# freemvmt/two-towers-overlords

Hardware: NVIDIA B200
Metric: train_triplets_per_sec (higher is better)
Workload: dtype f32 (bf16x3 tensor-core projection)

## Files before the change

### two-towers-overlords_b200/csrc/tt_chain_sm100.cu

```cuda
#include <stdlib.h>

#include "tt_ptx.cuh"
#include "tt_step_ws.cuh"
#include "tt_tma.cuh"

namespace tt {

namespace {

using namespace ptx;

constexpr int BM = 128, BN = 128, BK = 64;
constexpr int kMaxStages = 6;
constexpr int kAcc = 4;
constexpr int kEpiThreads = 256;
constexpr int kThreads = 64 + kEpiThreads;
constexpr uint32_t kABytes = BM * BK * 2, kBBytes = BN * BK * 2, kStageBytes = kABytes + kBBytes;
constexpr int kSplitPad = 66;
constexpr int kRowStage = 3072;
constexpr int kTermPitch = 48;
constexpr int kTermBlock = 32 * kTermPitch;
constexpr int kF32Pitch = 80;
constexpr int kCsBytes = 2 * 8 * 64 * 4;
constexpr int kStagingBytes = kCsBytes  + 8 * kRowStage  + 64;
static_assert(2 * 64 * kSplitPad * 2 <= 8 * kRowStage, "split tiles overlay the row staging");
constexpr size_t chain_smem(int stages) { return (size_t)stages * kStageBytes + 1024 + 256 + kStagingBytes; }
constexpr float kCosEps = 1e-8f;
constexpr long long kSpinLimit = 4000000000ll;

enum { T_S = 0, T_T, T_F1, T_F2L, T_DZ, T_DX, T_DW2, T_DW1, T_G, T_COUNT };

struct TowerMaps {
  CUtensorMap x[3], w1[3];
  CUtensorMap h[2], w2[2];
  CUtensorMap dy[2];
  CUtensorMap dz[2], w1k[2];
  CUtensorMap dyk[2], hk[2];
  CUtensorMap dzk[2], xk[2];
};

struct SplitJobC {
  const float* X;
  bf16 *hi, *lo, *lo2;
  int R, C;
  int f4_0;
};

struct alignas(64) ChainParams {
  TowerMaps tm[2];
  int B, H, P, RTB, NC, NCH, NCF, ldt, dcol;
  int pairs, terms, pairs1, terms1;
  int kcb, nch[2], kbt[2];
  int off[T_COUNT + 1];
  int stages, n_sj, n_split_f4, n_split_f4_w1;
  int nS;
  int krot;
  int use_pdl;
  SplitJobC sj[6];
  float margin, inv_batch, grad_scale;
  const float *b1[2], *b2[2];
  float *h, *y, *dy, *dz1, *dxhat, *stats, *loss;
  bf16 *h_hi, *h_lo, *dy_hi, *dy_lo, *dz_hi, *dz_lo;
  float *part2, *part1;
  float *dW1[2], *db1[2], *dW2[2], *db2[2];
  float *stat_part, *cs1, *cs2, *hinge_part, *ybuf;
  unsigned* ctr;
  int n_counters;
  double* adam_state;
  float *adam_p, *adam_g, *adam_m, *adam_v;
  float lr, beta1, beta2, eps;
  unsigned total_signals, dw2_signals;
  unsigned long long* trace;
};

__device__ __forceinline__ unsigned ld_acquire(const unsigned* p) {
  unsigned v;
  asm volatile("ld.acquire.gpu.global.u32 %0, [%1];" : "=r"(v) : "l"(p) : "memory");
  return v;
}
__device__ __forceinline__ void signal(unsigned* p) {
  asm volatile("red.release.gpu.global.add.u32 [%0], 1;" ::"l"(p) : "memory");
}
__device__ __forceinline__ void fence_proxy_async() { asm volatile("fence.proxy.async;" ::: "memory"); }
__device__ __forceinline__ unsigned ld_relaxed(const unsigned* p) {
  unsigned v;
  asm volatile("ld.relaxed.gpu.global.u32 %0, [%1];" : "=r"(v) : "l"(p) : "memory");
  return v;
}
__device__ __forceinline__ void wait_counter(const unsigned* p, unsigned target) {
  if (ld_relaxed(p) < target) {
    const long long t0 = clock64();
    while (ld_relaxed(p) < target) {
      __nanosleep(32);
      if (clock64() - t0 > kSpinLimit) __trap();
    }
  }
  asm volatile("fence.acq_rel.gpu;" ::: "memory");
}
__device__ __forceinline__ void epi_bar() { asm volatile("bar.sync 1, 256;" ::: "memory"); }

struct Task {
  int type, i;
};
__device__ __forceinline__ Task decode(const ChainParams& p, int idx) {
  int t = 0;
#pragma unroll
  for (int k = 1; k < T_COUNT; ++k)
    if (idx >= p.off[k]) t = k;
  return Task{t, idx - p.off[t]};
}

struct RowTile {
  int r, seg, t, trow, grow, valid;
};
__device__ __forceinline__ RowTile row_tile(const ChainParams& p, int u) {
  RowTile rt;
  rt.r = u / 3;
  rt.seg = u - 3 * rt.r;
  rt.t = rt.seg != 0;
  rt.trow = (rt.seg == 2 ? p.B : 0) + rt.r * BM;
  rt.grow = rt.seg * p.B + rt.r * BM;
  rt.valid = min(BM, p.B - rt.r * BM);
  return rt;
}

struct Sub {
  const CUtensorMap *a, *b;
  int terms, pairs, m0, n0, kb0, nkb;
  int bn;
  int amn, bmn;
};
__device__ __forceinline__ int n_subs(int type) {
  return (type == T_S || type == T_T || type == T_G) ? 0 : 1;
}

__device__ __forceinline__ void dw_chunk(const ChainParams& p, int ci, int& t, int& j) {
  t = ci >= p.nch[0];
  j = ci - (t ? p.nch[0] : 0);
}

__device__ __forceinline__ Sub get_sub(const ChainParams& p, Task tk, int k) {
  Sub s;
  s.terms = p.terms;
  s.pairs = p.pairs;
  s.kb0 = 0;
  s.bn = BN;
  s.amn = s.bmn = 0;
  switch (tk.type) {
    case T_F1: {
      const RowTile rt = row_tile(p, tk.i / p.NC);
      s.a = p.tm[rt.t].x; s.b = p.tm[rt.t].w1;
      s.terms = p.terms1; s.pairs = p.pairs1;
// ... 99 lines not shown
  for (int j = 0; j < 2; ++j) {
    const float keep = h4 ? b[2 + j] : b[j], send = h4 ? b[j] : b[2 + j];
    c[j] = keep + __shfl_xor_sync(0xffffffffu, send, 4);
  }
  const float keep = h2 ? c[1] : c[0], send = h2 ? c[0] : c[1];
  float d = keep + __shfl_xor_sync(0xffffffffu, send, 2);
  d += __shfl_xor_sync(0xffffffffu, d, 1);
  return d;
}

__device__ __forceinline__ void store16(float* dst, const float (&v)[16]) {
  float4* d = reinterpret_cast<float4*>(dst);
#pragma unroll
  for (int j = 0; j < 4; ++j) d[j] = make_float4(v[4 * j], v[4 * j + 1], v[4 * j + 2], v[4 * j + 3]);
}

__device__ __forceinline__ void split16(const float (&v)[16], bf16 (&hi)[16], bf16 (&lo)[16]) {
#pragma unroll
  for (int j = 0; j < 16; ++j) split_bf16(v[j], hi[j], lo[j]);
}
__device__ __forceinline__ void stage16(uint8_t* blk, int lane, const bf16 (&x)[16]) {
  uint4* d = reinterpret_cast<uint4*>(blk + lane * kTermPitch);
  d[0] = reinterpret_cast<const uint4*>(x)[0];
  d[1] = reinterpret_cast<const uint4*>(x)[1];
}
__device__ __forceinline__ void flush16(const uint8_t* blk, int lane, bf16* g, size_t row0, int n, int ld, int vr) {
#pragma unroll
  for (int it = 0; it < 2; ++it) {
    const int r = it * 16 + (lane >> 1), sg = lane & 1;
    if (r < vr)
      *reinterpret_cast<uint4*>(g + (row0 + r) * ld + n + sg * 8) =
          *reinterpret_cast<const uint4*>(blk + r * kTermPitch + sg * 16);
  }
}
__device__ __forceinline__ void stage_f32(uint8_t* blk, int lane, const float (&v)[16]) {
  float4* d = reinterpret_cast<float4*>(blk + lane * kF32Pitch);
#pragma unroll
  for (int j = 0; j < 4; ++j) d[j] = make_float4(v[4 * j], v[4 * j + 1], v[4 * j + 2], v[4 * j + 3]);
}
__device__ __forceinline__ void flush_f32(const uint8_t* blk, int lane, float* g, size_t row0, int n, size_t ld, int vr) {
#pragma unroll
  for (int it = 0; it < 4; ++it) {
    const int r = it * 8 + (lane >> 2), sg = lane & 3;
    if (r < vr)
      *reinterpret_cast<float4*>(g + (row0 + r) * ld + n + sg * 4) =
          *reinterpret_cast<const float4*>(blk + r * kF32Pitch + sg * 16);
  }
}

struct EpiCtx {
  uint32_t tmem_base;
  uint64_t *acc_full, *acc_empty;
  float* cs_s;
  bf16* sp_s;
  float* hs_s;
  uint8_t* rs;
  int we, q, hf, lane, tid;
  int ab;
  uint32_t aph;
  unsigned long long* trace;
  int tslot, tidx;
};

__device__ __forceinline__ void trace_ev(EpiCtx& e, int kind) {
  if (e.trace && e.tid == 0 && e.tslot < kTraceSlots) {
    unsigned long long t;
    asm volatile("mov.u64 %0, %globaltimer;" : "=l"(t));
    e.trace[e.tslot * 2] = ((unsigned long long)e.tidx << 2) | (unsigned long long)kind;
    e.trace[e.tslot * 2 + 1] = t;
    ++e.tslot;
  }
}

__device__ __forceinline__ uint32_t acc_addr(const EpiCtx& e, int buf, int chunk) {
  return e.tmem_base + ((uint32_t)(e.q * 32) << 16) + (uint32_t)(buf * BN + e.hf * 64 + chunk * 16);
}
__device__ __forceinline__ void acc_advance(EpiCtx& e, int n) {
  e.ab += n;
  if (e.ab >= kAcc) {
    e.ab -= kAcc;
    e.aph ^= 1u;
  }
}
__device__ __forceinline__ void publish(const EpiCtx& e) {
  fence_proxy_async();
  __threadfence();
  epi_bar();
}

__device__ __forceinline__ void stage_cs(const EpiCtx& e, int slot, int chunk, float d) {
  if ((e.lane & 1) == 0) e.cs_s[(slot * 8 + e.we) * 64 + chunk * 16 + (e.lane >> 1)] = d;
}
__device__ __forceinline__ float reduce_cs(const EpiCtx& e, int slot, int col, int cw = 64) {
  const int hf = col / cw, cc = col - hf * cw;
  float s = 0.f;
#pragma unroll
  for (int quarter = 0; quarter < 4; ++quarter) s += e.cs_s[(slot * 8 + hf * 4 + ((quarter - 2) & 3)) * 64 + cc];
  return s;
}

__device__ __forceinline__ uint32_t pack_bf16(bf16 a, bf16 b) {
  return (uint32_t)__bfloat16_as_ushort(a) | ((uint32_t)__bfloat16_as_ushort(b) << 16);
}

__device__ void epi_split(const ChainParams& p, EpiCtx& e, int task_i) {
  const int nS = p.nS;
  if (task_i == 0 && e.tid == 0 && p.adam_state) {
    const double t = p.adam_state[0];
    p.adam_state[0] = t + 1.0;
    p.adam_state[1] = (t == 0.0 ? 1.0 : p.adam_state[1]) * (double)p.beta1;
    p.adam_state[2] = (t == 0.0 ? 1.0 : p.adam_state[2]) * (double)p.beta2;
  }
  constexpr int U = 4;
  const int gstride = nS * kEpiThreads;
  for (int part = 0; part < 2; ++part) {
    const int lo_i = part ? p.n_split_f4_w1 : 0, hi_i = part ? p.n_split_f4 : p.n_split_f4_w1;
    for (int base = lo_i + task_i * kEpiThreads + e.tid; base < hi_i; base += U * gstride) {
      float4 v[U];
      int ji[U], li[U];
#pragma unroll
      for (int u = 0; u < U; ++u) {
        const int i = base + u * gstride;
        ji[u] = -1;
        if (i < hi_i) {
          int j = 0;
          for (int k = 1; k < p.n_sj; ++k)
            if (i >= p.sj[k].f4_0) j = k;
          ji[u] = j;
          li[u] = i - p.sj[j].f4_0;
          v[u] = __ldg(reinterpret_cast<const float4*>(p.sj[j].X) + li[u]);
        }
      }
#pragma unroll
      for (int u = 0; u < U; ++u) {
        if (ji[u] < 0) continue;
        const SplitJobC& J = p.sj[ji[u]];
        const float x[4] = {v[u].x, v[u].y, v[u].z, v[u].w};
        bf16 h[4], l[4];
#pragma unroll
        for (int k = 0; k < 4; ++k) split_bf16(x[k], h[k], l[k]);
        reinterpret_cast<uint2*>(J.hi)[li[u]] = make_uint2(pack_bf16(h[0], h[1]), pack_bf16(h[2], h[3]));
        reinterpret_cast<uint2*>(J.lo)[li[u]] = make_uint2(pack_bf16(l[0], l[1]), pack_bf16(l[2], l[3]));
        if (J.lo2) {
          bf16 m[4];
#pragma unroll
          for (int k = 0; k < 4; ++k)
            m[k] = __float2bfloat16_rn((x[k] - __bfloat162float(h[k])) - __bfloat162float(l[k]));
          reinterpret_cast<uint2*>(J.lo2)[li[u]] = make_uint2(pack_bf16(m[0], m[1]), pack_bf16(m[2], m[3]));
        }
      }
    }
    if (part == 0) {
      publish(e);
      if (e.tid == 0) signal(p.ctr + 0);
    }
  }
  publish(e);
  if (e.tid == 0) signal(p.ctr + 2);
}

__device__ __forceinline__ int warp_valid_rows(const EpiCtx& e, int valid) { return max(0, min(32, valid - e.q * 32)); }

__device__ void epi_f1(const ChainParams& p, EpiCtx& e, int task_i) {
  const RowTile rt = row_tile(p, task_i / p.NC);
  const int n0 = (task_i % p.NC) * BN;
  mbar_wait(&e.acc_full[e.ab], e.aph);
  tc_fence_after();
  trace_ev(e, 2);
  const int row = e.q * 32 + e.lane;
  const bool ok = row < rt.valid;
  const int vr = warp_valid_rows(e, rt.valid);
  const size_t wrow0 = (size_t)rt.grow + e.q * 32;
  const float* bias = p.b1[rt.t];
  for (int ch = 0; ch < 4; ++ch) {
    const int n = n0 + e.hf * 64 + ch * 16;
    if (n >= p.P) break;
    float v[16];
    tmem_ld16(acc_addr(e, e.ab, ch), v);
#pragma unroll
    for (int j = 0; j < 16; ++j) v[j] = fmaxf(v[j] + __ldg(bias + n + j), 0.f);
    alignas(16) bf16 hi[16], lo[16];
    split16(v, hi, lo);
    stage16(e.rs, e.lane, hi);
    stage16(e.rs + kTermBlock, e.lane, lo);
    if (ok && p.h) store16(p.h + (wrow0 + e.lane) * p.P + n, v);
    __syncwarp();
    flush16(e.rs, e.lane, p.h_hi, wrow0, n, p.P, vr);
    flush16(e.rs + kTermBlock, e.lane, p.h_lo, wrow0, n, p.P, vr);
    __syncwarp();
  }
  tc_fence_before();
  mbar_arrive(&e.acc_empty[e.ab]);
  acc_advance(e, 1);
  publish(e);
  if (e.tid == 0) signal(h_ready(p) + rt.seg * p.RTB + rt.r);
}

__device__ void epi_f2l(const ChainParams& p, EpiCtx& e, int task_i) {
  const int seg = task_i % 3, rc = task_i / 3, r = rc / p.NCF, c = rc % p.NCF, n0 = c * 64;
  const int valid = min(BM, p.B - r * BM);
  const int row = e.q * 32 + e.lane;
  const bool ok = row < valid;
  const int vr = warp_valid_rows(e, valid);
  const int trip = r * BM + row;
  const size_t wrow0 = (size_t)seg * p.B + (size_t)r * BM + e.q * 32;
  mbar_wait(&e.acc_full[e.ab], e.aph);
  tc_fence_after();
  trace_ev(e, 2);
  const uint32_t accb = e.tmem_base + ((uint32_t)(e.q * 32) << 16) + (uint32_t)(e.ab * BN + e.hf * 32);
  const float* bias = p.b2[seg != 0];
  float* X = p.ybuf + (size_t)rc * 3 * 64 * 128;
  float own[32];
#pragma unroll
  for (int ch = 0; ch < 2; ++ch) {
    const int col = e.hf * 32 + ch * 16;
    float v[16];
    tmem_ld16(accb + ch * 16, v);
#pragma unroll
    for (int j = 0; j < 16; ++j) {
      v[j] += __ldg(bias + n0 + col + j);
      own[ch * 16 + j] = v[j];
      X[((size_t)(seg * 64 + col + j)) * 128 + row] = v[j];
    }
    if (p.y && ok) store16(p.y + ((size_t)seg * p.B + trip) * p.P + n0 + col, v);
  }
  tc_fence_before();
  mbar_arrive(&e.acc_empty[e.ab]);
  acc_advance(e, 1);
  __threadfence();
  epi_bar();
  if (e.tid == 0) {
    signal(y_ready(p) + rc);
    wait_counter(y_ready(p) + rc, 3u);
  }
  epi_bar();
  const int s1 = seg == 0 ? 1 : 0, s2 = seg == 2 ? 1 : 2;
  float f1[32], f2[32];
  {
    const float* x1 = X + (size_t)(s1 * 64 + e.hf * 32) * 128 + row;
    const float* x2 = X + (size_t)(s2 * 64 + e.hf * 32) * 128 + row;
#pragma unroll
    for (int j = 0; j < 32; ++j) {
      f1[j] = __ldcg(x1 + (size_t)j * 128);
      f2[j] = __ldcg(x2 + (size_t)j * 128);
    }
  }
  float qq = 0.f, pp = 0.f, nn = 0.f, qp = 0.f, qn = 0.f;
#pragma unroll
  for (int j = 0; j < 32; ++j) {
    const float a = seg == 0 ? own[j] : f1[j];
    const float b = seg == 0 ? f1[j] : (seg == 1 ? own[j] : f2[j]);
    const float d = seg == 2 ? own[j] : f2[j];
    qq = fmaf(a, a, qq);
    pp = fmaf(b, b, pp);
    nn = fmaf(d, d, nn);
    qp = fmaf(a, b, qp);
    qn = fmaf(a, d, qn);
  }
  const int nslots = p.NCF;
  float* xs = e.cs_s;
  if (seg == 0 && e.hf == 1) {
    xs[row] = qq; xs[128 + row] = pp; xs[256 + row] = nn; xs[384 + row] = qp; xs[512 + row] = qn;
  }
  epi_bar();
  if (seg == 0 && e.hf == 0) {
    float* sp = p.stat_part + ((size_t)(r * nslots + c) * 5) * 128 + row;
    sp[0] = qq + xs[row]; sp[128] = pp + xs[128 + row]; sp[256] = nn + xs[256 + row]; sp[384] = qp + xs[384 + row];
    sp[512] = qn + xs[512 + row];
    __threadfence();
  }
  epi_bar();
  if (e.tid == 0) {
    if (seg == 0) signal(stat_ready(p) + r);
    wait_counter(stat_ready(p) + r, (unsigned)p.NCF);
  }
  epi_bar();
  trace_ev(e, 3);
  qq = pp = nn = qp = qn = 0.f;
  for (int s0 = 0; s0 < nslots; s0 += 4) {
    float v[4][5];
#pragma unroll
    for (int u = 0; u < 4; ++u) {
      const float* sp = p.stat_part + ((size_t)(r * nslots + min(s0 + u, nslots - 1)) * 5) * 128 + row;
#pragma unroll
      for (int w = 0; w < 5; ++w) v[u][w] = __ldcg(sp + 128 * w);
    }
#pragma unroll
    for (int u = 0; u < 4; ++u)
      if (s0 + u < nslots) {
        qq += v[u][0]; pp += v[u][1]; nn += v[u][2]; qp += v[u][3]; qn += v[u][4];
      }
  }
  const float nq = sqrtf(qq), np_ = sqrtf(pp), nn_ = sqrtf(nn);
  const float cq = fmaxf(nq, kCosEps), cp = fmaxf(np_, kCosEps), cn = fmaxf(nn_, kCosEps);
  const float cos_p = qp / (cq * cp), cos_n = qn / (cq * cn);
  const float hinge = ok ? fmaxf((1.f - cos_p) - (1.f - cos_n) + p.margin, 0.f) : 0.f;
  const float gh = (hinge > 0.f) ? p.grad_scale * p.inv_batch : 0.f;
  const float a_qp = -gh / (cq * cp), a_qn = gh / (cq * cn);
  float c_own, c1, c2;
  if (seg == 0) {
    c_own = -((nq > kCosEps) ? (-gh * cos_p + gh * cos_n) / (cq * nq) : 0.f); c1 = a_qp; c2 = a_qn;
  } else if (seg == 1) {
    c_own = -((np_ > kCosEps) ? (-gh * cos_p) / (cp * np_) : 0.f); c1 = a_qp; c2 = 0.f;
  } else {
    c_own = -((nn_ > kCosEps) ? (gh * cos_n) / (cn * nn_) : 0.f); c1 = a_qn; c2 = 0.f;
  }
  if (seg == 0 && c == 0 && e.hf == 0) {
    if (ok) {
      float* s = p.stats + (size_t)trip * 8;
      s[0] = cos_p; s[1] = cos_n; s[2] = hinge; s[3] = nq; s[4] = np_; s[5] = nn_; s[6] = qp; s[7] = qn;
    }
    const float hsum = warp_sum(hinge);
    if (e.lane == 0) e.hs_s[e.q] = hsum;
  }
  uint8_t* blk_hi = e.rs;
  uint8_t* blk_lo = e.rs + kTermBlock;
#pragma unroll
  for (int ch = 0; ch < 2; ++ch) {
    const int n = n0 + e.hf * 32 + ch * 16;
    float g[16];
#pragma unroll
    for (int j = 0; j < 16; ++j)
      g[j] = ok ? (c_own * own[ch * 16 + j] + c1 * f1[ch * 16 + j] + c2 * f2[ch * 16 + j]) : 0.f;
    alignas(16) bf16 hi[16], lo[16];
    split16(g, hi, lo);
    stage16(blk_hi, e.lane, hi);
    stage16(blk_lo, e.lane, lo);
    if (ok && p.dy) store16(p.dy + ((size_t)seg * p.B + trip) * p.P + n, g);
    __syncwarp();
    flush16(blk_hi, e.lane, p.dy_hi, wrow0, n, p.P, vr);
    flush16(blk_lo, e.lane, p.dy_lo, wrow0, n, p.P, vr);
    __syncwarp();
    stage_cs(e, 0, ch, colsum16(g, e.lane));
  }
  epi_bar();
  if (e.tid < 64) p.cs2[(size_t)(seg * p.RTB + r) * p.P + n0 + e.tid] = reduce_cs(e, 0, e.tid, 32);
  if (seg == 0 && c == 0 && e.tid == 0) p.hinge_part[r] = (e.hs_s[0] + e.hs_s[1]) + (e.hs_s[2] + e.hs_s[3]);
  publish(e);
  if (e.tid == 0) {
    signal(dy_ready(p) + seg * p.RTB + r);
    signal(p.ctr + 1);
  }
}

__device__ void epi_dz(const ChainParams& p, EpiCtx& e, int task_i) {
  const RowTile rt = row_tile(p, task_i / p.NC);
  const int n0 = (task_i % p.NC) * BN;
  mbar_wait(&e.acc_full[e.ab], e.aph);
  tc_fence_after();
  trace_ev(e, 2);
  const int row = e.q * 32 + e.lane;
  const bool ok = row < rt.valid;
  const int vr = warp_valid_rows(e, rt.valid);
  const size_t wrow0 = (size_t)rt.grow + e.q * 32;
  for (int ch = 0; ch < 4; ++ch) {
    const int n = n0 + e.hf * 64 + ch * 16;
    if (n >= p.P) break;
    float v[16];
    tmem_ld16(acc_addr(e, e.ab, ch), v);
    const size_t o = (wrow0 + e.lane) * p.P + n;
    if (ok) {
      alignas(16) bf16 g[16];
      reinterpret_cast<uint4*>(g)[0] = __ldcg(reinterpret_cast<const uint4*>(p.h_hi + o));
      reinterpret_cast<uint4*>(g)[1] = __ldcg(reinterpret_cast<const uint4*>(p.h_hi + o) + 1);
#pragma unroll
      for (int j = 0; j < 16; ++j) v[j] = __bfloat162float(g[j]) > 0.f ? v[j] : 0.f;
      if (p.dz1) store16(p.dz1 + o, v);
    } else {
#pragma unroll
      for (int j = 0; j < 16; ++j) v[j] = 0.f;
    }
    alignas(16) bf16 hi[16], lo[16];
    split16(v, hi, lo);
    stage16(e.rs, e.lane, hi);
    stage16(e.rs + kTermBlock, e.lane, lo);
    __syncwarp();
    flush16(e.rs, e.lane, p.dz_hi, wrow0, n, p.P, vr);
    flush16(e.rs + kTermBlock, e.lane, p.dz_lo, wrow0, n, p.P, vr);
    __syncwarp();
    stage_cs(e, 0, ch, colsum16(v, e.lane));
  }
  tc_fence_before();
  mbar_arrive(&e.acc_empty[e.ab]);
  acc_advance(e, 1);
  epi_bar();
  if (e.tid < BN && n0 + e.tid < p.P)
    p.cs1[(size_t)(rt.seg * p.RTB + rt.r) * p.P + n0 + e.tid] = reduce_cs(e, 0, e.tid);
  publish(e);
  if (e.tid == 0) {
    signal(dz_ready(p) + rt.seg * p.RTB + rt.r);
    signal(p.ctr + 1);
  }
}

__device__ __forceinline__ void epi_store_f32(const ChainParams& p, EpiCtx& e, float* g, size_t wrow0, int n0, int N,
                                              size_t ld, int vr) {
  for (int ch = 0; ch < 4; ++ch) {
    const int n = n0 + e.hf * 64 + ch * 16;
    if (n >= N) break;
    float v[16];
    tmem_ld16(acc_addr(e, e.ab, ch), v);
    stage_f32(e.rs, e.lane, v);
    __syncwarp();
    flush_f32(e.rs, e.lane, g, wrow0, n, ld, vr);
    __syncwarp();
  }
}

__device__ void epi_dx(const ChainParams& p, EpiCtx& e, int task_i) {
  const RowTile rt = row_tile(p, task_i / p.NCH);
  const int n0 = (task_i % p.NCH) * BN;
  mbar_wait(&e.acc_full[e.ab], e.aph);
  tc_fence_after();
  trace_ev(e, 2);
  epi_store_f32(p, e, p.dxhat, (size_t)rt.grow + e.q * 32, n0, p.H, p.H, warp_valid_rows(e, rt.valid));
  tc_fence_before();
  mbar_arrive(&e.acc_empty[e.ab]);
  acc_advance(e, 1);
}

__device__ void epi_dw(const ChainParams& p, EpiCtx& e, Task tk) {
  const bool two = tk.type == T_DW2;
  const int N = two ? p.P : p.H, ntn = two ? p.NC : p.NCH, nt_ = p.NC * ntn;
  const int ci = tk.i / nt_, tile = tk.i % nt_;
  const int m0 = (tile / ntn) * BM, n0 = (tile % ntn) * BN;
  float* part = (two ? p.part2 : p.part1) + (size_t)ci * p.P * N;
  mbar_wait(&e.acc_full[e.ab], e.aph);
  tc_fence_after();
  trace_ev(e, 2);
  epi_store_f32(p, e, part, (size_t)m0 + e.q * 32, n0, N, N, warp_valid_rows(e, p.P - m0));
  tc_fence_before();
  mbar_arrive(&e.acc_empty[e.ab]);
  acc_advance(e, 1);
  __threadfence();
  epi_bar();
  if (e.tid == 0) {
    if (two) signal(p.ctr + 5);
    signal(p.ctr + 1);
  }
}

__device__ __forceinline__ float4 add4(float4 a, float4 b) { return make_float4(a.x + b.x, a.y + b.y, a.z + b.z, a.w + b.w); }

struct AdamCoef {
  float step_size, bc2_sqrt;
};
__device__ __forceinline__ float adam1(const ChainParams& p, const AdamCoef& k, float g, float& m, float& v, float w) {
  m = m + (g - m) * (1.f - p.beta1);
  v = v * p.beta2 + (1.f - p.beta2) * g * g;
  const float denom = sqrtf(v) / k.bc2_sqrt + p.eps;
  return w - k.step_size * (m / denom);
}
__device__ __forceinline__ void emit4(const ChainParams& p, const AdamCoef& k, float4* dst, float4 g) {
  *dst = g;
  if (!p.adam_p) return;
  const size_t off = reinterpret_cast<float*>(dst) - p.adam_g;
  float4 m = *reinterpret_cast<float4*>(p.adam_m + off), v = *reinterpret_cast<float4*>(p.adam_v + off);
  float4 w = *reinterpret_cast<float4*>(p.adam_p + off);
  w.x = adam1(p, k, g.x, m.x, v.x, w.x);
  w.y = adam1(p, k, g.y, m.y, v.y, w.y);
  w.z = adam1(p, k, g.z, m.z, v.z, w.z);
  w.w = adam1(p, k, g.w, m.w, v.w, w.w);
  *reinterpret_cast<float4*>(p.adam_m + off) = m;
  *reinterpret_cast<float4*>(p.adam_v + off) = v;
  *reinterpret_cast<float4*>(p.adam_p + off) = w;
}
__device__ __forceinline__ void emit1(const ChainParams& p, const AdamCoef& k, float* dst, float g) {
  *dst = g;
  if (!p.adam_p) return;
  const size_t off = dst - p.adam_g;
  float m = p.adam_m[off], v = p.adam_v[off];
  p.adam_p[off] = adam1(p, k, g, m, v, p.adam_p[off]);
  p.adam_m[off] = m;
  p.adam_v[off] = v;
}

__device__ void epi_grad(const ChainParams& p, EpiCtx& e, int task_i) {
  if (e.tid == 0) wait_counter(p.ctr + 5, p.dw2_signals);
  epi_bar();
  trace_ev(e, 2);
  AdamCoef k{0.f, 1.f};
  if (p.adam_p) {
    const volatile double* st = p.adam_state;
    k.step_size = (float)((double)p.lr / (1.0 - st[1]));
    k.bc2_sqrt = (float)sqrt(1.0 - st[2]);
  }
  const int nG = p.off[T_COUNT] - p.off[T_G];
  volatile int* claim_s = reinterpret_cast<volatile int*>(e.cs_s);
  int round = 0;
  auto sum_pairs = [&](unsigned* claim, const float* part, float* const (&dW)[2], size_t n4) {
    auto locate = [&](size_t item, const float4*& src, float4*& dst, int& nch) {
      const int t = item >= n4;
      const size_t i = item - (t ? n4 : 0);
      nch = p.nch[t];
      src = reinterpret_cast<const float4*>(part) + (size_t)(t ? p.nch[0] : 0) * n4 + i;
      dst = reinterpret_cast<float4*>(dW[t]) + i;
    };
    const size_t ntot = 2 * n4;
    const int nchunks = (int)((ntot + 2 * kEpiThreads - 1) / (2 * kEpiThreads));
    for (;;) {
      if (e.tid == 0) claim_s[round & 1] = (int)atomicAdd(claim, 1u);
      epi_bar();
      const int c = claim_s[round & 1];
      ++round;
      if (c >= nchunks) break;
      const size_t it = (size_t)c * 2 * kEpiThreads + e.tid;
      if (it >= ntot) continue;
      const float4* src[2];
      float4* dst[2];
      int nch[2];
      const bool two = it + kEpiThreads < ntot;
      locate(it, src[0], dst[0], nch[0]);
      locate(two ? it + kEpiThreads : it, src[1], dst[1], nch[1]);
      float4 acc[2] = {make_float4(0.f, 0.f, 0.f, 0.f), make_float4(0.f, 0.f, 0.f, 0.f)};
      const int nmax = max(nch[0], nch[1]);
      for (int j = 0; j < nmax; j += 4) {
        float4 t[2][4];
#pragma unroll
        for (int u = 0; u < 2; ++u)
#pragma unroll
          for (int c4 = 0; c4 < 4; ++c4)
            t[u][c4] = (j + c4 < nch[u]) ? __ldcg(src[u] + (size_t)(j + c4) * n4) : make_float4(0.f, 0.f, 0.f, 0.f);
#pragma unroll
        for (int u = 0; u < 2; ++u)
#pragma unroll
          for (int c4 = 0; c4 < 4; ++c4)
            if (j + c4 < nch[u]) acc[u] = add4(acc[u], t[u][c4]);
      }
      emit4(p, k, dst[0], acc[0]);
      if (two) emit4(p, k, dst[1], acc[1]);
    }
  };
  sum_pairs(p.ctr + 6, p.part2, p.dW2, (size_t)p.P * p.P / 4);
  if (e.tid == 0) wait_counter(p.ctr + 1, p.total_signals);
  epi_bar();
  sum_pairs(p.ctr + 7, p.part1, p.dW1, (size_t)p.P * p.H / 4);
  {
    const int nout = 4 * p.P;
    const int gw = task_i * 8 + e.we, nw = nG * 8;
    for (int o = gw; o < nout; o += nw) {
      const int which = o / p.P, n = o - which * p.P, t = which & 1;
      const float* src;
      int cnt;
      if (which < 2) {
        src = p.cs2 + (size_t)(t ? p.RTB : 0) * p.P + n;
        cnt = t ? 2 * p.RTB : p.RTB;
      } else {
        src = p.cs1 + (size_t)(t ? p.RTB : 0) * p.P + n;
        cnt = t ? 2 * p.RTB : p.RTB;
      }
      float s = 0.f;
      for (int r = e.lane; r < cnt; r += 32) s += __ldcg(src + (size_t)r * p.P);
      s = warp_sum(s);
      if (e.lane == 0) emit1(p, k, (which < 2 ? p.db2[t] : p.db1[t]) + n, s);
    }
  }
  if (task_i == 0 && e.tid == 0) {
    float s = 0.f;
    for (int r = 0; r < p.RTB; ++r) s += __ldcg(p.hinge_part + r);
    *p.loss = s * p.inv_batch;
  }
  epi_bar();
  if (e.tid == 0) {
    __threadfence();
    if (atomicAdd(p.ctr + 4, 1u) == (unsigned)nG - 1u) {
      for (int i = 0; i < p.n_counters; ++i) p.ctr[i] = 0u;
    }
  }
}

__global__ void __launch_bounds__(kThreads, 1) chain_kernel(const __grid_constant__ ChainParams p) {
  extern __shared__ uint8_t smem_raw[];
  const int warp = threadIdx.x >> 5, lane = threadIdx.x & 31;
  const uint32_t raw = smem_u32(smem_raw);
  uint8_t* smem = smem_raw + (((raw + 1023u) & ~1023u) - raw);
  const int NS = p.stages;
  uint64_t* full = reinterpret_cast<uint64_t*>(smem + NS * kStageBytes);
  uint64_t* empty = full + kMaxStages;
  uint64_t* acc_full = empty + kMaxStages;
  uint64_t* acc_empty = acc_full + kAcc;
  uint32_t* tmem_slot = reinterpret_cast<uint32_t*>(acc_empty + kAcc);
  uint8_t* staging = smem + NS * kStageBytes + 256;

  if (threadIdx.x == 0) {
    for (int s = 0; s < NS; ++s) {
      mbar_init(&full[s], 1);
      mbar_init(&empty[s], 1);
    }
    for (int b = 0; b < kAcc; ++b) {
      mbar_init(&acc_full[b], 1);
      mbar_init(&acc_empty[b], kEpiThreads);
    }
    fence_barrier_init();
  }
  if (warp == 1) {
    tmem_alloc(tmem_slot, kAcc * BN);
    tmem_relinquish();
  }
  tc_fence_before();
  __syncthreads();
  tc_fence_after();
  const uint32_t tmem_base = *tmem_slot;
  const int n_tasks = p.off[T_COUNT];

  if (warp == 0) {
    if (elect_one()) {
      int s = 0;
      uint32_t ph = 0;
      if (p.use_pdl) pdl_wait();
      for (int idx = blockIdx.x; idx < n_tasks; idx += gridDim.x) {
        const Task tk = decode(p, idx);
        const int ns = n_subs(tk.type);
        if (ns == 0) continue;
        wait_deps(p, tk);
        fence_proxy_async();
        for (int k = 0; k < ns; ++k) {
          const Sub sb = get_sub(p, tk, k);
          int kb = sb.kb0 + (p.krot ? (int)(blockIdx.x % (unsigned)sb.nkb) : 0);
          for (int kbi = 0; kbi < sb.nkb; ++kbi, kb = (kb + 1 == sb.kb0 + sb.nkb) ? sb.kb0 : kb + 1) {
            for (int j = 0; j < sb.terms; ++j) {
              mbar_wait(&empty[s], ph ^ 1u);
              mbar_arrive_expect_tx(&full[s], kABytes + (uint32_t)sb.bn * BK * 2);
              uint8_t* sa = smem + s * kStageBytes;
              uint8_t* sbm = sa + kABytes;
              if (sb.amn) {
                tma_load_2d(sa, &sb.a[j], &full[s], sb.m0, kb * BK);
                tma_load_2d(sa + kABytes / 2, &sb.a[j], &full[s], sb.m0 + 64, kb * BK);
              } else {
                tma_load_2d(sa, &sb.a[j], &full[s], kb * BK, sb.m0);
              }
              if (sb.bmn) {
                tma_load_2d(sbm, &sb.b[j], &full[s], sb.n0, kb * BK);
                tma_load_2d(sbm + kBBytes / 2, &sb.b[j], &full[s], sb.n0 + 64, kb * BK);
              } else {
                tma_load_2d(sbm, &sb.b[j], &full[s], kb * BK, sb.n0);
              }
              if (++s == NS) {
                s = 0;
                ph ^= 1u;
              }
            }
          }
        }
      }
// ... 1 lines not shown
  } else if (warp == 1) {
    if (elect_one()) {
      constexpr uint32_t idesc128 = make_idesc_bf16(BM, BN), idesc64 = make_idesc_bf16(BM, 64);
      const uint32_t ring = smem_u32(smem);
      int s = 0, ab = 0;
      uint32_t ph = 0, aph = 0;
      for (int idx = blockIdx.x; idx < n_tasks; idx += gridDim.x) {
        const Task tk = decode(p, idx);
        const int ns = n_subs(tk.type);
        for (int k = 0; k < ns; ++k) {
          const Sub sb = get_sub(p, tk, k);
          const uint32_t idesc = (sb.bn == BN ? idesc128 : idesc64) | ((uint32_t)sb.amn << 15) | ((uint32_t)sb.bmn << 16);
          const uint64_t a_step = sb.amn ? 128 : 2, b_step = sb.bmn ? 128 : 2;
          mbar_wait(&acc_empty[ab], aph ^ 1u);
          tc_fence_after();
          const uint32_t acc = tmem_base + (uint32_t)(ab * BN);
          for (int kbi = 0; kbi < sb.nkb; ++kbi) {
            uint32_t slot_addr[3];
            int slot_id[3];
            for (int j = 0; j < sb.terms; ++j) {
              mbar_wait(&full[s], ph);
              slot_id[j] = s;
              slot_addr[j] = ring + (uint32_t)s * kStageBytes;
              if (++s == NS) {
                s = 0;
                ph ^= 1u;
              }
            }
            tc_fence_after();
            for (int pair = 0; pair < sb.pairs; ++pair) {
              const int ai = (0x201100 >> (4 * pair)) & 3, bi = (0x021010 >> (4 * pair)) & 3;
              const uint64_t da = sb.amn ? make_smem_desc_sw128_mn(slot_addr[ai], kABytes / 2) : make_smem_desc_sw128(slot_addr[ai]),
                             db = sb.bmn ? make_smem_desc_sw128_mn(slot_addr[bi] + kABytes, kBBytes / 2)
                                         : make_smem_desc_sw128(slot_addr[bi] + kABytes);
#pragma unroll
              for (int kk = 0; kk < BK / 16; ++kk)
                mma_bf16(acc, da + a_step * kk, db + b_step * kk, idesc, (kbi | pair | kk) != 0);
            }
            for (int j = 0; j < sb.terms; ++j) mma_commit(&empty[slot_id[j]]);
          }
          mma_commit(&acc_full[ab]);
          if (++ab == kAcc) {
            ab = 0;
            aph ^= 1u;
          }
        }
      }
    }
  } else {
    EpiCtx e;
    e.tmem_base = tmem_base;
    e.acc_full = acc_full;
    e.acc_empty = acc_empty;
    e.cs_s = reinterpret_cast<float*>(staging);
    e.sp_s = reinterpret_cast<bf16*>(staging + kCsBytes);
    e.rs = staging + kCsBytes + (warp - 2) * kRowStage;
    e.hs_s = reinterpret_cast<float*>(staging + kCsBytes + 8 * kRowStage);
    e.we = warp - 2;
    e.q = warp & 3;
    e.hf = e.we >> 2;
    e.lane = lane;
    e.tid = threadIdx.x - 64;
    e.ab = 0;
    e.aph = 0;
    e.trace = p.trace ? p.trace + (size_t)blockIdx.x * kTraceSlots * 2 : nullptr;
    e.tslot = 0;
    for (int idx = blockIdx.x; idx < n_tasks; idx += gridDim.x) {
      const Task tk = decode(p, idx);
      e.tidx = idx;
      trace_ev(e, 0);
      switch (tk.type) {
        case T_S:
          epi_split(p, e, tk.i);
          if (p.use_pdl) pdl_wait();
          break;
        case T_F1: epi_f1(p, e, tk.i); break;
        case T_F2L: epi_f2l(p, e, tk.i); break;
        case T_DZ: epi_dz(p, e, tk.i); break;
        case T_DX: epi_dx(p, e, tk.i); break;
        case T_DW2:
        case T_DW1: epi_dw(p, e, tk); break;
        default: epi_grad(p, e, tk.i); break;
      }
      trace_ev(e, 1);
    }
  }
  tc_fence_before();
  __syncthreads();
  if (warp == 1) tmem_dealloc(tmem_base, kAcc * BN);
}

int chain_stages() {
  static int v = -1;
  if (v < 0) {
    const char* e = getenv("TT_CHAIN_STAGES");
    v = e ? atoi(e) : 0;
    if (v < 3 || v > kMaxStages) v = 5;
  }
  return v;
}

int chain_debug_out() {
  const char* e = getenv("TT_CHAIN_FP32_OUT");
  return e ? atoi(e) : 0;
}

int map_terms(CUtensorMap* m, int n, const bf16* const* ptr, uint64_t rows, uint64_t cols, uint64_t ld,
              uint32_t box_rows = BM) {
  for (int i = 0; i < n; ++i) {
    const bf16* base = ptr[i] ? ptr[i] : ptr[0];
    int rc = make_map_bf16_kmajor(&m[i], base, rows, cols, ld, box_rows);
    if (rc) return rc;
  }
  return 0;
}

}

bool chain_enabled() {
  const char* e = getenv("TT_CHAIN");
  return e ? atoi(e) != 0 : true;
// ... 144 lines not shown
```

### two-towers-overlords_b200/csrc/tt_step_ws.cuh

```cuda
#pragma once
#include "tt_simt.cuh"
#include "tt_sm100.cuh"

namespace tt {

using bf16 = __nv_bfloat16;
static inline int round64(int x) { return (x + 63) / 64 * 64; }

struct StepWs {
  int ldt, dcol;
  bf16 *x_hi, *x_lo, *x_lo2, *xt_hi, *xt_lo;
  bf16 *h_hi, *h_lo, *ht_hi, *ht_lo;
  bf16 *dy_hi, *dy_lo, *dyt_hi, *dyt_lo;
  bf16 *dz_hi, *dz_lo, *dzt_hi, *dzt_lo;
  bf16 *w1_hi[2], *w1_lo[2], *w1_lo2[2], *w1t_hi[2], *w1t_lo[2];
  bf16 *w2_hi[2], *w2_lo[2], *w2t_hi[2], *w2t_lo[2];
  float *dz1, *partial, *partial2, *colsum, *colsum2, *loss_scratch;
  float *stat_part, *cs1, *cs2, *hinge_part, *ybuf;
  unsigned* counters;
  int n_counters;
  unsigned long long* trace;
};
constexpr int kTraceSlots = 64, kTraceCtas = 160;

static inline size_t carve_step(char* base, int B, int H, int P, int train_table, StepWs* out) {
  char* p = base;
  StepWs w{};
  w.dcol = round64(B);
  w.ldt = w.dcol + round64(2 * B);
  const size_t R = (size_t)3 * B;
  w.x_hi = ws_take<bf16>(p, R * H); w.x_lo = ws_take<bf16>(p, R * H); w.x_lo2 = ws_take<bf16>(p, R * H);
  w.xt_hi = ws_take<bf16>(p, (size_t)H * w.ldt); w.xt_lo = ws_take<bf16>(p, (size_t)H * w.ldt);
  w.h_hi = ws_take<bf16>(p, R * P); w.h_lo = ws_take<bf16>(p, R * P);
  w.ht_hi = ws_take<bf16>(p, (size_t)P * w.ldt); w.ht_lo = ws_take<bf16>(p, (size_t)P * w.ldt);
  w.dy_hi = ws_take<bf16>(p, R * P); w.dy_lo = ws_take<bf16>(p, R * P);
  w.dyt_hi = ws_take<bf16>(p, (size_t)P * w.ldt); w.dyt_lo = ws_take<bf16>(p, (size_t)P * w.ldt);
  w.dz_hi = ws_take<bf16>(p, R * P); w.dz_lo = ws_take<bf16>(p, R * P);
  w.dzt_hi = ws_take<bf16>(p, (size_t)P * w.ldt); w.dzt_lo = ws_take<bf16>(p, (size_t)P * w.ldt);
  for (int t = 0; t < 2; ++t) {
    w.w1_hi[t] = ws_take<bf16>(p, (size_t)P * H); w.w1_lo[t] = ws_take<bf16>(p, (size_t)P * H);
    w.w1_lo2[t] = ws_take<bf16>(p, (size_t)P * H);
    w.w1t_hi[t] = ws_take<bf16>(p, (size_t)P * H); w.w1t_lo[t] = ws_take<bf16>(p, (size_t)P * H);
    w.w2_hi[t] = ws_take<bf16>(p, (size_t)P * P); w.w2_lo[t] = ws_take<bf16>(p, (size_t)P * P);
    w.w2t_hi[t] = ws_take<bf16>(p, (size_t)P * P); w.w2t_lo[t] = ws_take<bf16>(p, (size_t)P * P);
  }
  w.dz1 = ws_take<float>(p, R * P);
  w.partial = ws_take<float>(p, (size_t)2 * 32 * P * max(P, H));
  w.partial2 = ws_take<float>(p, (size_t)2 * 32 * P * P);
  w.colsum = ws_take<float>(p, (size_t)2 * kColsumSlices * P);
  w.colsum2 = ws_take<float>(p, (size_t)2 * kColsumSlices * P);
  w.loss_scratch = ws_take<float>(p, (size_t)(B + 3) / 4 + 8);
  {
    const int RTB = (B + 127) / 128, NC = (P + 127) / 128;
    w.stat_part = ws_take<float>(p, (size_t)RTB * 2 * (P / 64 + 1) * 5 * 128);
    w.cs1 = ws_take<float>(p, (size_t)3 * RTB * P);
    w.cs2 = ws_take<float>(p, (size_t)3 * RTB * P);
    w.ybuf = ws_take<float>(p, (size_t)3 * RTB * 128 * P);
    w.hinge_part = ws_take<float>(p, (size_t)RTB + 8);
    w.n_counters = 10 * RTB + 8 + RTB * (P / 64 + 1);
    w.counters = ws_take<unsigned>(p, (size_t)w.n_counters);
    w.trace = ws_take<unsigned long long>(p, (size_t)kTraceCtas * kTraceSlots * 2);
  }
  (void)train_table;
  if (out) *out = w;
  return (size_t)(p - base) + 256;
}


}
```

Measured before the change: 8.553 million.

## Split epilogue warps into two independent groups alternating accumulator tiles

```diff
diff --git a/two-towers-overlords_b200/csrc/tt_chain_sm100.cu b/two-towers-overlords_b200/csrc/tt_chain_sm100.cu
--- a/two-towers-overlords_b200/csrc/tt_chain_sm100.cu
+++ b/two-towers-overlords_b200/csrc/tt_chain_sm100.cu
@@ -14,6 +14,7 @@
 constexpr int kMaxStages = 6;
 constexpr int kAcc = 4;
 constexpr int kEpiThreads = 256;
+constexpr int kGroupThreads = 128;
 constexpr int kThreads = 64 + kEpiThreads;
 constexpr uint32_t kABytes = BM * BK * 2, kBBytes = BN * BK * 2, kStageBytes = kABytes + kBBytes;
 constexpr int kSplitPad = 66;
@@ -21,10 +22,11 @@
 constexpr int kTermPitch = 48;
 constexpr int kTermBlock = 32 * kTermPitch;
 constexpr int kF32Pitch = 80;
-constexpr int kCsBytes = 2 * 8 * 64 * 4;
-constexpr int kStagingBytes = kCsBytes  + 8 * kRowStage  + 64;
+constexpr int kCsBytes = 2 * 4 * 128 * 4;
+constexpr int kStagingBytes = kCsBytes  + 8 * kRowStage  + 64 ;
 static_assert(2 * 64 * kSplitPad * 2 <= 8 * kRowStage, "split tiles overlay the row staging");
 constexpr size_t chain_smem(int stages) { return (size_t)stages * kStageBytes + 1024 + 256 + kStagingBytes; }
+static_assert(chain_smem(kMaxStages) <= 227 * 1024, "every ring depth up to kMaxStages fits the shared memory of a CTA");
 constexpr float kCosEps = 1e-8f;
 constexpr long long kSpinLimit = 4000000000ll;
 
@@ -97,7 +99,8 @@
   }
   asm volatile("fence.acq_rel.gpu;" ::: "memory");
 }
-__device__ __forceinline__ void epi_bar() { asm volatile("bar.sync 1, 256;" ::: "memory"); }
+__device__ __forceinline__ void grp_bar(int g) { asm volatile("bar.sync %0, 128;" ::"r"(1 + g) : "memory"); }
+__device__ __forceinline__ void joint_bar() { asm volatile("bar.sync 3, 256;" ::: "memory"); }
 
 struct Task {
   int type, i;
@@ -303,10 +306,10 @@
   uint32_t tmem_base;
   uint64_t *acc_full, *acc_empty;
   float* cs_s;
-  bf16* sp_s;
   float* hs_s;
+  int* claim_s;
   uint8_t* rs;
-  int we, q, hf, lane, tid;
+  int we, q, g, lane, tid, gt;
   int ab;
   uint32_t aph;
   unsigned long long* trace;
@@ -314,7 +317,7 @@
 };
 
 __device__ __forceinline__ void trace_ev(EpiCtx& e, int kind) {
-  if (e.trace && e.tid == 0 && e.tslot < kTraceSlots) {
+  if (e.trace && e.gt == 0 && e.tslot < kTraceSlots / 2) {
     unsigned long long t;
     asm volatile("mov.u64 %0, %globaltimer;" : "=l"(t));
     e.trace[e.tslot * 2] = ((unsigned long long)e.tidx << 2) | (unsigned long long)kind;
@@ -324,10 +327,12 @@
 }
 
 __device__ __forceinline__ uint32_t acc_addr(const EpiCtx& e, int buf, int chunk) {
-  return e.tmem_base + ((uint32_t)(e.q * 32) << 16) + (uint32_t)(buf * BN + e.hf * 64 + chunk * 16);
-}
-__device__ __forceinline__ void acc_advance(EpiCtx& e, int n) {
-  e.ab += n;
+  return e.tmem_base + ((uint32_t)(e.q * 32) << 16) + (uint32_t)(buf * BN + chunk * 16);
+}
+__device__ __forceinline__ void acc_release(EpiCtx& e) {
+  tc_fence_before();
+  mbar_arrive(&e.acc_empty[e.ab]);
+  e.ab += 2;
   if (e.ab >= kAcc) {
     e.ab -= kAcc;
     e.aph ^= 1u;
@@ -336,17 +341,21 @@
 __device__ __forceinline__ void publish(const EpiCtx& e) {
   fence_proxy_async();
   __threadfence();
-  epi_bar();
-}
-
-__device__ __forceinline__ void stage_cs(const EpiCtx& e, int slot, int chunk, float d) {
-  if ((e.lane & 1) == 0) e.cs_s[(slot * 8 + e.we) * 64 + chunk * 16 + (e.lane >> 1)] = d;
-}
-__device__ __forceinline__ float reduce_cs(const EpiCtx& e, int slot, int col, int cw = 64) {
-  const int hf = col / cw, cc = col - hf * cw;
+  grp_bar(e.g);
+}
+__device__ __forceinline__ void publish_joint() {
+  fence_proxy_async();
+  __threadfence();
+  joint_bar();
+}
+
+__device__ __forceinline__ void stage_cs(const EpiCtx& e, int chunk, float d) {
+  if ((e.lane & 1) == 0) e.cs_s[e.q * 128 + chunk * 16 + (e.lane >> 1)] = d;
+}
+__device__ __forceinline__ float reduce_cs(const EpiCtx& e, int col) {
   float s = 0.f;
 #pragma unroll
-  for (int quarter = 0; quarter < 4; ++quarter) s += e.cs_s[(slot * 8 + hf * 4 + ((quarter - 2) & 3)) * 64 + cc];
+  for (int quarter = 0; quarter < 4; ++quarter) s += e.cs_s[quarter * 128 + col];
   return s;
 }
 
@@ -402,11 +411,11 @@
       }
     }
     if (part == 0) {
-      publish(e);
+      publish_joint();
       if (e.tid == 0) signal(p.ctr + 0);
     }
   }
-  publish(e);
+  publish_joint();
   if (e.tid == 0) signal(p.ctr + 2);
 }
 
@@ -423,8 +432,8 @@
   const int vr = warp_valid_rows(e, rt.valid);
   const size_t wrow0 = (size_t)rt.grow + e.q * 32;
   const float* bias = p.b1[rt.t];
-  for (int ch = 0; ch < 4; ++ch) {
-    const int n = n0 + e.hf * 64 + ch * 16;
+  for (int ch = 0; ch < BN / 16; ++ch) {
+    const int n = n0 + ch * 16;
     if (n >= p.P) break;
     float v[16];
     tmem_ld16(acc_addr(e, e.ab, ch), v);
@@ -440,11 +449,26 @@
     flush16(e.rs + kTermBlock, e.lane, p.h_lo, wrow0, n, p.P, vr);
     __syncwarp();
   }
-  tc_fence_before();
-  mbar_arrive(&e.acc_empty[e.ab]);
-  acc_advance(e, 1);
+  acc_release(e);
   publish(e);
-  if (e.tid == 0) signal(h_ready(p) + rt.seg * p.RTB + rt.r);
+  if (e.gt == 0) signal(h_ready(p) + rt.seg * p.RTB + rt.r);
+}
+
+template <int W>
+__device__ __forceinline__ void f2l_load(const float* X, int seg, int c, int row, float (&f1)[W], float (&f2)[W]) {
+  const int s1 = seg == 0 ? 1 : 0, s2 = seg == 2 ? 1 : 2;
+  const float* x1 = X + (size_t)(s1 * 64 + c * W) * 128 + row;
+  const float* x2 = X + (size_t)(s2 * 64 + c * W) * 128 + row;
+#pragma unroll
+  for (int j = 0; j < W; ++j) {
+    f1[j] = __ldcg(x1 + (size_t)j * 128);
+    f2[j] = __ldcg(x2 + (size_t)j * 128);
+  }
+}
+__device__ __forceinline__ void f2l_own(const EpiCtx& e, const float* bias, int ch, float (&v)[16]) {
+  tmem_ld16(acc_addr(e, e.ab, ch), v);
+#pragma unroll
+  for (int j = 0; j < 16; ++j) v[j] += __ldg(bias + ch * 16 + j);
 }
 
 __device__ void epi_f2l(const ChainParams& p, EpiCtx& e, int task_i) {
@@ -458,76 +482,66 @@
   mbar_wait(&e.acc_full[e.ab], e.aph);
   tc_fence_after();
   trace_ev(e, 2);
-  const uint32_t accb = e.tmem_base + ((uint32_t)(e.q * 32) << 16) + (uint32_t)(e.ab * BN + e.hf * 32);
-  const float* bias = p.b2[seg != 0];
+  const float* bias = p.b2[seg != 0] + n0;
   float* X = p.ybuf + (size_t)rc * 3 * 64 * 128;
-  float own[32];
-#pragma unroll
-  for (int ch = 0; ch < 2; ++ch) {
-    const int col = e.hf * 32 + ch * 16;
+#pragma unroll
+  for (int ch = 0; ch < 4; ++ch) {
+    const int col = ch * 16;
     float v[16];
-    tmem_ld16(accb + ch * 16, v);
-#pragma unroll
-    for (int j = 0; j < 16; ++j) {
-      v[j] += __ldg(bias + n0 + col + j);
-      own[ch * 16 + j] = v[j];
-      X[((size_t)(seg * 64 + col + j)) * 128 + row] = v[j];
-    }
+    f2l_own(e, bias, ch, v);
+#pragma unroll
+    for (int j = 0; j < 16; ++j) X[((size_t)(seg * 64 + col + j)) * 128 + row] = v[j];
     if (p.y && ok) store16(p.y + ((size_t)seg * p.B + trip) * p.P + n0 + col, v);
   }
-  tc_fence_before();
-  mbar_arrive(&e.acc_empty[e.ab]);
-  acc_advance(e, 1);
   __threadfence();
-  epi_bar();
-  if (e.tid == 0) {
+  grp_bar(e.g);
+  if (e.gt == 0) {
     signal(y_ready(p) + rc);
     wait_counter(y_ready(p) + rc, 3u);
   }
-  epi_bar();
-  const int s1 = seg == 0 ? 1 : 0, s2 = seg == 2 ? 1 : 2;
-  float f1[32], f2[32];
-  {
-    const float* x1 = X + (size_t)(s1 * 64 + e.hf * 32) * 128 + row;
-    const float* x2 = X + (size_t)(s2 * 64 + e.hf * 32) * 128 + row;
-#pragma unroll
-    for (int j = 0; j < 32; ++j) {
-      f1[j] = __ldcg(x1 + (size_t)j * 128);
-      f2[j] = __ldcg(x2 + (size_t)j * 128);
-    }
-  }
-  float qq = 0.f, pp = 0.f, nn = 0.f, qp = 0.f, qn = 0.f;
-#pragma unroll
-  for (int j = 0; j < 32; ++j) {
-    const float a = seg == 0 ? own[j] : f1[j];
-    const float b = seg == 0 ? f1[j] : (seg == 1 ? own[j] : f2[j]);
-    const float d = seg == 2 ? own[j] : f2[j];
-    qq = fmaf(a, a, qq);
-    pp = fmaf(b, b, pp);
-    nn = fmaf(d, d, nn);
-    qp = fmaf(a, b, qp);
-    qn = fmaf(a, d, qn);
+  grp_bar(e.g);
+  float st[2][5];
+#pragma unroll
+  for (int h = 0; h < 2; ++h) {
+    float qq = 0.f, pp = 0.f, nn = 0.f, qp = 0.f, qn = 0.f;
+#pragma unroll 1
+    for (int k = 0; k < 2; ++k) {
+      float own[16], f1[16], f2[16];
+      f2l_load(X, seg, 2 * h + k, row, f1, f2);
+      f2l_own(e, bias, 2 * h + k, own);
+#pragma unroll
+      for (int j = 0; j < 16; ++j) {
+        const float a = seg == 0 ? own[j] : f1[j];
+        const float b = seg == 0 ? f1[j] : (seg == 1 ? own[j] : f2[j]);
+        const float d = seg == 2 ? own[j] : f2[j];
+        qq = fmaf(a, a, qq);
+        pp = fmaf(b, b, pp);
+        nn = fmaf(d, d, nn);
+        qp = fmaf(a, b, qp);
+        qn = fmaf(a, d, qn);
+      }
+    }
+    if (h == 0) {
+      st[0][0] = qq; st[0][1] = pp; st[0][2] = nn; st[0][3] = qp; st[0][4] = qn;
+    } else {
+      st[1][0] = qq; st[1][1] = pp; st[1][2] = nn; st[1][3] = qp; st[1][4] = qn;
+    }
   }
   const int nslots = p.NCF;
-  float* xs = e.cs_s;
-  if (seg == 0 && e.hf == 1) {
-    xs[row] = qq; xs[128 + row] = pp; xs[256 + row] = nn; xs[384 + row] = qp; xs[512 + row] = qn;
-  }
-  epi_bar();
-  if (seg == 0 && e.hf == 0) {
+  if (seg == 0) {
     float* sp = p.stat_part + ((size_t)(r * nslots + c) * 5) * 128 + row;
-    sp[0] = qq + xs[row]; sp[128] = pp + xs[128 + row]; sp[256] = nn + xs[256 + row]; sp[384] = qp + xs[384 + row];
-    sp[512] = qn + xs[512 + row];
+#pragma unroll
+    for (int w = 0; w < 5; ++w) sp[128 * w] = st[0][w] + st[1][w];
     __threadfence();
   }
-  epi_bar();
-  if (e.tid == 0) {
+  grp_bar(e.g);
+  if (e.gt == 0) {
     if (seg == 0) signal(stat_ready(p) + r);
     wait_counter(stat_ready(p) + r, (unsigned)p.NCF);
   }
-  epi_bar();
+  grp_bar(e.g);
   trace_ev(e, 3);
-  qq = pp = nn = qp = qn = 0.f;
+  float qq = 0.f, pp = 0.f, nn = 0.f, qp = 0.f, qn = 0.f;
   for (int s0 = 0; s0 < nslots; s0 += 4) {
     float v[4][5];
 #pragma unroll
@@ -556,7 +570,7 @@
   } else {
     c_own = -((nn_ > kCosEps) ? (gh * cos_n) / (cn * nn_) : 0.f); c1 = a_qn; c2 = 0.f;
   }
-  if (seg == 0 && c == 0 && e.hf == 0) {
+  if (seg == 0 && c == 0) {
     if (ok) {
       float* s = p.stats + (size_t)trip * 8;
       s[0] = cos_p; s[1] = cos_n; s[2] = hinge; s[3] = nq; s[4] = np_; s[5] = nn_; s[6] = qp; s[7] = qn;
@@ -566,13 +580,14 @@
   }
   uint8_t* blk_hi = e.rs;
   uint8_t* blk_lo = e.rs + kTermBlock;
-#pragma unroll
-  for (int ch = 0; ch < 2; ++ch) {
-    const int n = n0 + e.hf * 32 + ch * 16;
-    float g[16];
-#pragma unroll
-    for (int j = 0; j < 16; ++j)
-      g[j] = ok ? (c_own * own[ch * 16 + j] + c1 * f1[ch * 16 + j] + c2 * f2[ch * 16 + j]) : 0.f;
+#pragma unroll 1
+  for (int ch = 0; ch < 4; ++ch) {
+    const int n = n0 + ch * 16;
+    float f1[16], f2[16], g[16];
+    f2l_load(X, seg, ch, row, f1, f2);
+    f2l_own(e, bias, ch, g);
+#pragma unroll
+    for (int j = 0; j < 16; ++j) g[j] = ok ? (c_own * g[j] + c1 * f1[j] + c2 * f2[j]) : 0.f;
     alignas(16) bf16 hi[16], lo[16];
     split16(g, hi, lo);
     stage16(blk_hi, e.lane, hi);
@@ -582,13 +597,14 @@
     flush16(blk_hi, e.lane, p.dy_hi, wrow0, n, p.P, vr);
     flush16(blk_lo, e.lane, p.dy_lo, wrow0, n, p.P, vr);
     __syncwarp();
-    stage_cs(e, 0, ch, colsum16(g, e.lane));
-  }
-  epi_bar();
-  if (e.tid < 64) p.cs2[(size_t)(seg * p.RTB + r) * p.P + n0 + e.tid] = reduce_cs(e, 0, e.tid, 32);
-  if (seg == 0 && c == 0 && e.tid == 0) p.hinge_part[r] = (e.hs_s[0] + e.hs_s[1]) + (e.hs_s[2] + e.hs_s[3]);
+    stage_cs(e, ch, colsum16(g, e.lane));
+  }
+  acc_release(e);
+  grp_bar(e.g);
+  if (e.gt < 64) p.cs2[(size_t)(seg * p.RTB + r) * p.P + n0 + e.gt] = reduce_cs(e, e.gt);
+  if (seg == 0 && c == 0 && e.gt == 0) p.hinge_part[r] = (e.hs_s[0] + e.hs_s[1]) + (e.hs_s[2] + e.hs_s[3]);
   publish(e);
-  if (e.tid == 0) {
+  if (e.gt == 0) {
     signal(dy_ready(p) + seg * p.RTB + r);
     signal(p.ctr + 1);
   }
@@ -604,16 +620,25 @@
   const bool ok = row < rt.valid;
   const int vr = warp_valid_rows(e, rt.valid);
   const size_t wrow0 = (size_t)rt.grow + e.q * 32;
-  for (int ch = 0; ch < 4; ++ch) {
-    const int n = n0 + e.hf * 64 + ch * 16;
+  const uint4* gsrc = reinterpret_cast<const uint4*>(p.h_hi + (wrow0 + e.lane) * p.P + n0);
+  uint4 nx0 = make_uint4(0u, 0u, 0u, 0u), nx1 = nx0;
+  if (ok) {
+    nx0 = __ldcg(gsrc);
+    nx1 = __ldcg(gsrc + 1);
+  }
+  for (int ch = 0; ch < BN / 16; ++ch) {
+    const int n = n0 + ch * 16;
     if (n >= p.P) break;
+    alignas(16) uint4 gt[2] = {nx0, nx1};
+    if (ok && ch + 1 < BN / 16 && n + 16 < p.P) {
+      nx0 = __ldcg(gsrc + 2 * (ch + 1));
+      nx1 = __ldcg(gsrc + 2 * (ch + 1) + 1);
+    }
     float v[16];
     tmem_ld16(acc_addr(e, e.ab, ch), v);
     const size_t o = (wrow0 + e.lane) * p.P + n;
     if (ok) {
-      alignas(16) bf16 g[16];
-      reinterpret_cast<uint4*>(g)[0] = __ldcg(reinterpret_cast<const uint4*>(p.h_hi + o));
-      reinterpret_cast<uint4*>(g)[1] = __ldcg(reinterpret_cast<const uint4*>(p.h_hi + o) + 1);
+      const bf16* g = reinterpret_cast<const bf16*>(gt);
 #pragma unroll
       for (int j = 0; j < 16; ++j) v[j] = __bfloat162float(g[j]) > 0.f ? v[j] : 0.f;
       if (p.dz1) store16(p.dz1 + o, v);
@@ -629,16 +654,13 @@
     flush16(e.rs, e.lane, p.dz_hi, wrow0, n, p.P, vr);
     flush16(e.rs + kTermBlock, e.lane, p.dz_lo, wrow0, n, p.P, vr);
     __syncwarp();
-    stage_cs(e, 0, ch, colsum16(v, e.lane));
-  }
-  tc_fence_before();
-  mbar_arrive(&e.acc_empty[e.ab]);
-  acc_advance(e, 1);
-  epi_bar();
-  if (e.tid < BN && n0 + e.tid < p.P)
-    p.cs1[(size_t)(rt.seg * p.RTB + rt.r) * p.P + n0 + e.tid] = reduce_cs(e, 0, e.tid);
+    stage_cs(e, ch, colsum16(v, e.lane));
+  }
+  acc_release(e);
+  grp_bar(e.g);
+  if (n0 + e.gt < p.P) p.cs1[(size_t)(rt.seg * p.RTB + rt.r) * p.P + n0 + e.gt] = reduce_cs(e, e.gt);
   publish(e);
-  if (e.tid == 0) {
+  if (e.gt == 0) {
     signal(dz_ready(p) + rt.seg * p.RTB + rt.r);
     signal(p.ctr + 1);
   }
@@ -646,8 +668,8 @@
 
 __device__ __forceinline__ void epi_store_f32(const ChainParams& p, EpiCtx& e, float* g, size_t wrow0, int n0, int N,
                                               size_t ld, int vr) {
-  for (int ch = 0; ch < 4; ++ch) {
-    const int n = n0 + e.hf * 64 + ch * 16;
+  for (int ch = 0; ch < BN / 16; ++ch) {
+    const int n = n0 + ch * 16;
     if (n >= N) break;
     float v[16];
     tmem_ld16(acc_addr(e, e.ab, ch), v);
@@ -665,9 +687,7 @@
   tc_fence_after();
   trace_ev(e, 2);
   epi_store_f32(p, e, p.dxhat, (size_t)rt.grow + e.q * 32, n0, p.H, p.H, warp_valid_rows(e, rt.valid));
-  tc_fence_before();
-  mbar_arrive(&e.acc_empty[e.ab]);
-  acc_advance(e, 1);
+  acc_release(e);
 }
 
 __device__ void epi_dw(const ChainParams& p, EpiCtx& e, Task tk) {
@@ -680,12 +700,10 @@
   tc_fence_after();
   trace_ev(e, 2);
   epi_store_f32(p, e, part, (size_t)m0 + e.q * 32, n0, N, N, warp_valid_rows(e, p.P - m0));
-  tc_fence_before();
-  mbar_arrive(&e.acc_empty[e.ab]);
-  acc_advance(e, 1);
+  acc_release(e);
   __threadfence();
-  epi_bar();
-  if (e.tid == 0) {
+  grp_bar(e.g);
+  if (e.gt == 0) {
     if (two) signal(p.ctr + 5);
     signal(p.ctr + 1);
   }
@@ -728,7 +746,7 @@
 
 __device__ void epi_grad(const ChainParams& p, EpiCtx& e, int task_i) {
   if (e.tid == 0) wait_counter(p.ctr + 5, p.dw2_signals);
-  epi_bar();
+  joint_bar();
   trace_ev(e, 2);
   AdamCoef k{0.f, 1.f};
   if (p.adam_p) {
@@ -737,7 +755,7 @@
     k.bc2_sqrt = (float)sqrt(1.0 - st[2]);
   }
   const int nG = p.off[T_COUNT] - p.off[T_G];
-  volatile int* claim_s = reinterpret_cast<volatile int*>(e.cs_s);
+  volatile int* claim_s = e.claim_s;
   int round = 0;
   auto sum_pairs = [&](unsigned* claim, const float* part, float* const (&dW)[2], size_t n4) {
     auto locate = [&](size_t item, const float4*& src, float4*& dst, int& nch) {
@@ -751,7 +769,7 @@
     const int nchunks = (int)((ntot + 2 * kEpiThreads - 1) / (2 * kEpiThreads));
     for (;;) {
       if (e.tid == 0) claim_s[round & 1] = (int)atomicAdd(claim, 1u);
-      epi_bar();
+      joint_bar();
       const int c = claim_s[round & 1];
       ++round;
       if (c >= nchunks) break;
@@ -784,7 +802,7 @@
   };
   sum_pairs(p.ctr + 6, p.part2, p.dW2, (size_t)p.P * p.P / 4);
   if (e.tid == 0) wait_counter(p.ctr + 1, p.total_signals);
-  epi_bar();
+  joint_bar();
   sum_pairs(p.ctr + 7, p.part1, p.dW1, (size_t)p.P * p.H / 4);
   {
     const int nout = 4 * p.P;
@@ -811,7 +829,7 @@
     for (int r = 0; r < p.RTB; ++r) s += __ldcg(p.hinge_part + r);
     *p.loss = s * p.inv_batch;
   }
-  epi_bar();
+  joint_bar();
   if (e.tid == 0) {
     __threadfence();
     if (atomicAdd(p.ctr + 4, 1u) == (unsigned)nG - 1u) {
@@ -840,7 +858,7 @@
     }
     for (int b = 0; b < kAcc; ++b) {
       mbar_init(&acc_full[b], 1);
-      mbar_init(&acc_empty[b], kEpiThreads);
+      mbar_init(&acc_empty[b], kGroupThreads);
     }
     fence_barrier_init();
   }
@@ -948,21 +966,24 @@
     e.tmem_base = tmem_base;
     e.acc_full = acc_full;
     e.acc_empty = acc_empty;
-    e.cs_s = reinterpret_cast<float*>(staging);
-    e.sp_s = reinterpret_cast<bf16*>(staging + kCsBytes);
-    e.rs = staging + kCsBytes + (warp - 2) * kRowStage;
-    e.hs_s = reinterpret_cast<float*>(staging + kCsBytes + 8 * kRowStage);
     e.we = warp - 2;
     e.q = warp & 3;
-    e.hf = e.we >> 2;
+    e.g = e.we >> 2;
     e.lane = lane;
     e.tid = threadIdx.x - 64;
-    e.ab = 0;
+    e.gt = e.tid & (kGroupThreads - 1);
+    e.cs_s = reinterpret_cast<float*>(staging) + e.g * 4 * 128;
+    e.rs = staging + kCsBytes + (warp - 2) * kRowStage;
+    e.hs_s = reinterpret_cast<float*>(staging + kCsBytes + 8 * kRowStage) + e.g * 4;
+    e.claim_s = reinterpret_cast<int*>(staging + kCsBytes + 8 * kRowStage) + 8;
+    e.ab = e.g;
     e.aph = 0;
-    e.trace = p.trace ? p.trace + (size_t)blockIdx.x * kTraceSlots * 2 : nullptr;
+    e.trace = p.trace ? p.trace + ((size_t)blockIdx.x * kTraceSlots + e.g * (kTraceSlots / 2)) * 2 : nullptr;
     e.tslot = 0;
+    int n_acc = 0;
     for (int idx = blockIdx.x; idx < n_tasks; idx += gridDim.x) {
       const Task tk = decode(p, idx);
+      if (n_subs(tk.type) && (n_acc++ & 1) != e.g) continue;
       e.tidx = idx;
       trace_ev(e, 0);
       switch (tk.type) {
diff --git a/two-towers-overlords_b200/csrc/tt_step_ws.cuh b/two-towers-overlords_b200/csrc/tt_step_ws.cuh
--- a/two-towers-overlords_b200/csrc/tt_step_ws.cuh
+++ b/two-towers-overlords_b200/csrc/tt_step_ws.cuh
@@ -21,7 +21,7 @@
   int n_counters;
   unsigned long long* trace;
 };
-constexpr int kTraceSlots = 64, kTraceCtas = 160;
+constexpr int kTraceSlots = 128, kTraceCtas = 160;
 
 static inline size_t carve_step(char* base, int B, int H, int P, int train_table, StepWs* out) {
   char* p = base;
```

Result: no change. 8.559 million (median of 6 runs) (+0.1%).
